# emdgroup/tnmf

Measured on AMD Instinct MI355X. Metric: MU-iterations/sec, higher is better.
Workload: dtype f32

## Files before the change

### tnmf_amd/csrc/fft.h

```cpp
#pragma once
#include "common.h"

struct FftArgs {
    const void *src0, *src1, *src2;
    void *dst0, *dst1;
    long ps_src, ps_dst;
    int planes, rows, cols;
    int ld_src, ld_dst;
    int KX, KXP;
    int yoff, xoff;
    int N, M, C, Hy;
    int n0, ngroups, nper;
    int mgroups, mper;
    int clamp0;
    double reg;
};

enum FftOp {
    kFftRowsFwd = 0,
    kFftRowsInv,
    kFftRowsInv2,
    kFftRowsMu,
    kFftColsFwd,
    kFftColsInv,
    kFftContractR,
    kFftGradH,
    kFftGradW,
};

typedef int (*fft_run_fn)(int op, int dtype, const FftArgs *a, hipStream_t s);
#define TNMF_FFT_DECL(L) int fft_run_##L(int op, int dtype, const FftArgs *a, hipStream_t s)
TNMF_FFT_DECL(32);
TNMF_FFT_DECL(48);
TNMF_FFT_DECL(64);
TNMF_FFT_DECL(96);
TNMF_FFT_DECL(144);
TNMF_FFT_DECL(192);
TNMF_FFT_DECL(270);
TNMF_FFT_DECL(288);
TNMF_FFT_DECL(384);
TNMF_FFT_DECL(540);
TNMF_FFT_DECL(576);
#undef TNMF_FFT_DECL

bool mixed_has_reconstruct(const Geo &g, int dtype);
bool mixed_has_grad_W(const Geo &g, int dtype);
int mixed_reconstruct(const Geo &g, const void *Tsp, const void *WT, void *OT, int KX, int KXP, hipStream_t s);
int mixed_grad_W(const Geo &g, const void *Tsp, const void *VT, const void *RT, void *Gn, void *Gp, int KX, int KXP,
                 int ngroups, int nper, hipStream_t s);

#ifndef TNMF_MIX_W3_WAVES
#define TNMF_MIX_W3_WAVES 3
#endif
constexpr int kMixW3Atoms = 16, kMixW3Waves = TNMF_MIX_W3_WAVES, kMixW3MaxAy = 12;
constexpr long kMixW3MinBytes = 24L << 20;
constexpr int mix_w3_waves(int Ay) {
    const int w = Ay >= 8 ? 3 : (Ay >= 4 ? 4 : (Ay >= 2 ? 5 : 7));
    return kMixW3Waves < 3 ? kMixW3Waves : w;
}
bool mixed_grad_W3_takes(const Geo &g, int KXP);

int spectral_contract_R(const Geo &g, int dtype, const void *SH, const void *SW, void *SR, int Ly, int KX, int KXP,
                        hipStream_t s);
int spectral_grad_W(const Geo &g, int dtype, const void *SH, const void *SV, const void *SR, void *Gn, void *Gp, int Ly,
                    int KX, int KXP, int ngroups, int nper, hipStream_t s);

bool fft_has(const Geo &g, int dtype);
void fft_invalidate(tnmf_hip_ctx *ctx);
void fft_invalidate_H(tnmf_hip_ctx *ctx, const Geo &g, int dtype, const void *H);
void fft_bind(tnmf_hip_ctx *ctx, const Geo &g, int dtype, const void *H, const void *V);
void fft_unbind(tnmf_hip_ctx *ctx);
void fft_invalidate_W(tnmf_hip_ctx *ctx);
void fft_release(tnmf_hip_ctx *ctx);
int fft_reserve(tnmf_hip_ctx *ctx, const Geo &g, int dtype, bool with_window);

int fft_reconstruct(tnmf_hip_ctx *ctx, const Geo &g, int dtype, const void *W, const void *H, void *R, bool nonneg,
                    hipStream_t s);
int fft_grad_H(tnmf_hip_ctx *ctx, const Geo &g, int dtype, const void *V, const void *R, const void *W, void *neg,
               void *pos, hipStream_t s);
int fft_update_H(tnmf_hip_ctx *ctx, const Geo &g, int dtype, const void *V, const void *R, const void *W, void *H,
                 double reg, hipStream_t s);
int fft_grad_W(tnmf_hip_ctx *ctx, const Geo &g, int dtype, const void *V, const void *R, const void *H, void *neg,
               void *pos, bool nonneg, hipStream_t s);
```

### tnmf_amd/csrc/fft.hip

```cpp
#include <algorithm>
#include <cstdlib>

#include "fft.h"
#include "fft_engine.h"

namespace {

const int kLensY[] = {32, 48, 64, 96, 144, 192, 270, 288, 384, 576};
const int kLensX[] = {32, 48, 64, 96, 144, 192, 270, 288, 384, 540, 576};
constexpr int kMixMaxGroups = 128;

int pick_len(int h, int dtype, bool along_x, bool tall = false) {
    if (along_x || tall) {
        for (int L : kLensX)
            if (L >= h && (dtype == 0 || L <= 288)) return L;
        return 0;
    }
    for (int L : kLensY)
        if (L >= h && (dtype == 0 || L <= 288)) return L;
    return 0;
}

bool tall_columns(const tnmf_hip_ctx *ctx) { return ctx->path != TNMF_PATH_FFT; }

fft_run_fn lookup(int L) {
    switch (L) {
        case 32: return fft_run_32;
        case 48: return fft_run_48;
        case 64: return fft_run_64;
        case 96: return fft_run_96;
        case 144: return fft_run_144;
        case 192: return fft_run_192;
        case 270: return fft_run_270;
        case 288: return fft_run_288;
        case 384: return fft_run_384;
        case 540: return fft_run_540;
        case 576: return fft_run_576;
        default: return nullptr;
    }
}

bool use_mixed(const Geo &g, int dtype, bool grad_W);

struct Lay {
    int Ly, Lx, KX, KXP, ngroups, nper, chunk, mgroups, mper;
    fft_run_fn rowf, colf;
    size_t csz;
    size_t T, SH, Tn, Tp, SV, SR, Ts, VT, RT, SW, SWf, TW, TWr, Wt, Gn, Gp, Gs, Wo, total, total_no_window;
    size_t sT, sSH, sS, sD;
    bool resident;
};

void sample_groups(const Geo &g, int tiles, int *ngroups, int *nper) {
    int ng = cdiv(2048, g.M * tiles);
    if (ng > 16) ng = 16;
    if (ng > g.N) ng = g.N;
    if (ng < 1) ng = 1;
    *nper = cdiv(g.N > 0 ? g.N : 1, ng);
    *ngroups = cdiv(g.N > 0 ? g.N : 1, *nper);
}

bool make_layout(const tnmf_hip_ctx *ctx, const Geo &gfull, const Geo &g, int dtype, Lay *l) {
    l->Ly = pick_len(g.Hy, dtype, false, tall_columns(ctx));
    l->Lx = pick_len(g.Hx, dtype, true);
    if (!l->Ly || !l->Lx) return false;
    l->rowf = lookup(l->Lx);
    l->colf = lookup(l->Ly);
    l->KX = l->Lx / 2 + 1;
    l->KXP = (int)align_up((size_t)l->KX, 16);
    l->csz = dtype == 0 ? 8 : 16;
    const int tiles = cdiv(l->KX, l->Ly > 384 ? 8 : 16);
    int ngroups_full, nper_full;
    sample_groups(gfull, tiles, &ngroups_full, &nper_full);
    sample_groups(g, tiles, &l->ngroups, &l->nper);
    const size_t c = l->csz, kxp = (size_t)l->KXP;
    const size_t Nf = gfull.N > 0 ? gfull.N : 1;
    l->sT = (size_t)g.M * g.Hy * kxp * c;
    l->sSH = (size_t)g.M * l->Ly * kxp * c;
    l->sS = (size_t)g.C * l->Ly * kxp * c;
    l->sD = (size_t)g.C * g.Dy * kxp * c;
    size_t budget = (size_t)8 << 30;
    if (const char *e = tnmf_diag_env("TNMF_FFT_WINDOW_MB")) budget = (size_t)atol(e) << 20;
    long chunk_full = (long)(budget / (2 * l->sT));
    if (chunk_full < 1) chunk_full = 1;
    if (chunk_full > (long)Nf) chunk_full = (long)Nf;
    l->chunk = (int)(chunk_full > g.N && g.N > 0 ? g.N : chunk_full);
    int mg = cdiv(1024, l->chunk * cdiv(l->KX, 16) * 2);
    if (mg > g.M) mg = g.M;
    if (mg < 1) mg = 1;
    l->mper = cdiv(g.M, mg);
    l->mgroups = cdiv(g.M, l->mper);
    const size_t nSW = (size_t)g.M * g.C * l->Ly * kxp * c;
    size_t o = 0;
    auto take = [&o](size_t bytes) {
        const size_t at = o;
        o += align_up(bytes, 256);
        return at;
    };
    l->T = take(Nf * l->sT + (size_t)64 * kxp * c);
    l->resident = !(use_mixed(g, dtype, false) && use_mixed(g, dtype, true));
    l->SH = take(l->resident ? Nf * l->sSH : 0);
    l->SV = take(Nf * l->sS);
    l->SR = take(Nf * l->sS);
    l->Ts = take(Nf * l->sD);
    l->VT = take(Nf * l->sD);
    l->RT = take(Nf * l->sD);
    l->SW = take(nSW);
    l->SWf = take(nSW);
    l->TW = take((size_t)2 * g.M * g.C * g.Ay * kxp * c);
    l->TWr = take((size_t)g.M * g.C * g.Ay * kxp * c);
    l->Wt = take((size_t)2 * g.M * g.C * g.Ay * g.Ax * (c / 2));
    const size_t nG = std::max(nSW * ngroups_full, (size_t)kMixMaxGroups * g.M * g.C * g.Ay * kxp * c);
    l->Gn = take(nG);
    l->Gp = take(nG);
    l->Gs = take(nSW * 2);
    l->Wo = take((size_t)2 * g.M * g.C * g.Ay * g.Ax * (c / 2));
    l->total_no_window = o;
    const size_t nTc = (size_t)chunk_full * l->sT;
    l->Tn = take(nTc);
    l->Tp = take(nTc);
    l->total = o;
    return true;
}

void clear_flags(FftState &f) {
    f.W_ok = false;
    std::fill(f.T_ok.begin(), f.T_ok.end(), 0);
    std::fill(f.SH_ok.begin(), f.SH_ok.end(), 0);
    std::fill(f.V_ok.begin(), f.V_ok.end(), 0);
    std::fill(f.SV_ok.begin(), f.SV_ok.end(), 0);
}

int ensure_ws(tnmf_hip_ctx *ctx, size_t bytes) {
    FftState &f = ctx->fft;
    if (bytes <= f.ws_bytes) return TNMF_OK;
    if (f.failed_bytes && bytes >= f.failed_bytes) return TNMF_E_WORKSPACE;
    const size_t want = align_up(bytes, 1 << 20);
    void *bigger = nullptr;
    if (hipMalloc(&bigger, want) != hipSuccess) {
        (void)hipGetLastError();
        bigger = nullptr;
        if (!f.ws) {
            f.failed_bytes = bytes;
            return TNMF_E_WORKSPACE;
        }
    }
    if (f.ws) {
        TNMF_HIP_TRY(hipDeviceSynchronize());
        TNMF_HIP_TRY(hipFree(f.ws));
        f.ws = nullptr;
        f.ws_bytes = 0;
        clear_flags(f);
    }
    if (!bigger && hipMalloc(&bigger, want) != hipSuccess) {
        (void)hipGetLastError();
        f.failed_bytes = bytes;
        return TNMF_E_WORKSPACE;
    }
    f.ws = bigger;
    f.ws_bytes = want;
    clear_flags(f);
    return TNMF_OK;
}

inline char *at(tnmf_hip_ctx *ctx, size_t off) { return static_cast<char *>(ctx->fft.ws) + off; }

#define CHECK(rc_expr)                  \
    do {                                \
        const int _rc = (rc_expr);      \
        if (_rc != TNMF_OK) return _rc; \
    } while (0)

template <typename T>
__global__ void k_fft_prep_W(const T *W, T *out0, T *out1, int planes, int Ay, int Ax, double scale) {
    const int i = blockIdx.x * blockDim.x + threadIdx.x, per = Ay * Ax;
    if (i >= planes * per) return;
    const int p = i / per, r = i - p * per, ay = r / Ax, ax = r - ay * Ax;
    const T v = (T)(scale * (double)W[i]);
    out0[i] = v;
    out1[(long)p * per + (Ay - 1 - ay) * Ax + (Ax - 1 - ax)] = v;
}

template <typename T>
__global__ __launch_bounds__(64) void k_fft_sum_groups(const cplx<T> *parts0, const cplx<T> *parts1, cplx<T> *out0,
                                                      cplx<T> *out1, long count, int ngroups, double scale) {
    const long i = (long)blockIdx.x * blockDim.x + threadIdx.x;
    if (i >= count) return;
    const cplx<T> *parts = blockIdx.y ? parts1 : parts0;
    double re = 0, im = 0;
    int gidx = 0;
    for (; gidx + 4 <= ngroups; gidx += 4) {
        cplx<T> v[4];
#pragma unroll
        for (int k = 0; k < 4; ++k) v[k] = parts[(gidx + k) * count + i];
#pragma unroll
        for (int k = 0; k < 4; ++k) {
            re += (double)v[k].x;
            im += (double)v[k].y;
        }
    }
    for (; gidx < ngroups; ++gidx) {
        const cplx<T> v = parts[gidx * count + i];
        re += (double)v.x;
        im += (double)v.y;
    }
    (blockIdx.y ? out1 : out0)[i] = {(T)(re * scale), (T)(im * scale)};
}

template <typename T>
__global__ void k_fft_flip_out(const T *in, T *out, int planes, int Ay, int Ax, int clamp0) {
    const int i = blockIdx.x * blockDim.x + threadIdx.x, per = Ay * Ax;
    if (i >= planes * per) return;
    const int p = i / per, r = i - p * per, ay = r / Ax, ax = r - ay * Ax;
    T v = in[(long)p * per + (Ay - 1 - ay) * Ax + (Ax - 1 - ax)];
    if (clamp0) v = v < (T)0 ? (T)0 : v;
    out[i] = v;
}

FftArgs base_args(const Geo &g, const Lay &l) {
    FftArgs a = {};
    a.KX = l.KX;
    a.KXP = l.KXP;
    a.N = g.N;
    a.M = g.M;
    a.C = g.C;
    a.Hy = g.Hy;
    return a;
}

int forward_planes(const Geo &g, const Lay &l, int dtype, const void *src, int planes, int rows, int cols, void *Ttmp,
                   void *S, hipStream_t s) {
    FftArgs a = base_args(g, l);
    a.src0 = src;
    a.dst0 = Ttmp;
    a.planes = planes;
    a.rows = rows;
    a.cols = cols;
    a.ld_src = cols;
    a.ps_src = (long)rows * cols;
    a.ps_dst = (long)rows * l.KXP;
    CHECK(l.rowf(kFftRowsFwd, dtype, &a, s));
    FftArgs b = base_args(g, l);
    b.src0 = Ttmp;
    b.dst0 = S;
    b.planes = planes;
    b.rows = rows;
    return l.colf(kFftColsFwd, dtype, &b, s);
}

bool use_mixed(const Geo &g, int dtype, bool grad_W) {
    static const bool off = tnmf_diag_env("TNMF_FFT_NO_MIXED") != nullptr;
    return !off && (grad_W ? mixed_has_grad_W(g, dtype) : mixed_has_reconstruct(g, dtype));
}

bool use_resident(const Lay &l) {
    static const bool off = tnmf_diag_env("TNMF_FFT_NO_RESIDENT") != nullptr;
    return l.resident && !off;
}

int scaled_W(tnmf_hip_ctx *ctx, const Geo &g, const Lay &l, int dtype, const void *W, double scale, hipStream_t s) {
    const int planes = g.M * g.C, n = planes * g.Ay * g.Ax;
    char *wt = at(ctx, l.Wt);
    const size_t half = (size_t)n * (l.csz / 2);
    if (dtype == 0)
        hipLaunchKernelGGL(k_fft_prep_W<float>, dim3(cdiv(n, 256)), dim3(256), 0, s, (const float *)W, (float *)wt,
                           (float *)(wt + half), planes, g.Ay, g.Ax, scale);
    else
        hipLaunchKernelGGL(k_fft_prep_W<double>, dim3(cdiv(n, 256)), dim3(256), 0, s, (const double *)W, (double *)wt,
                           (double *)(wt + half), planes, g.Ay, g.Ax, scale);
    TNMF_LAUNCH_CHECK();
    return TNMF_OK;
}

int spectra_W(tnmf_hip_ctx *ctx, const Geo &g, const Lay &l, int dtype, const void *W, bool plain, bool flipped,
              hipStream_t s) {
    const int planes = g.M * g.C, per = g.Ay * g.Ax, n = planes * per;
    const double scale = 1.0 / ((double)l.Ly * l.Lx);
    char *wt = at(ctx, l.Wt);
    const size_t half = (size_t)n * (l.csz / 2);
    if (dtype == 0)
        hipLaunchKernelGGL(k_fft_prep_W<float>, dim3(cdiv(n, 256)), dim3(256), 0, s, (const float *)W, (float *)wt,
                           (float *)(wt + half), planes, g.Ay, g.Ax, scale);
    else
        hipLaunchKernelGGL(k_fft_prep_W<double>, dim3(cdiv(n, 256)), dim3(256), 0, s, (const double *)W, (double *)wt,
                           (double *)(wt + half), planes, g.Ay, g.Ax, scale);
    TNMF_LAUNCH_CHECK();
    if (plain) CHECK(forward_planes(g, l, dtype, wt, planes, g.Ay, g.Ax, at(ctx, l.TW), at(ctx, l.SW), s));
    if (flipped) CHECK(forward_planes(g, l, dtype, wt + half, planes, g.Ay, g.Ax, at(ctx, l.TW), at(ctx, l.SWf), s));
    return TNMF_OK;
}


inline size_t esz_of(int dtype) { return dtype == 0 ? 4 : 8; }

bool same_shape(const Geo &a, const Geo &b) {
    return a.M == b.M && a.C == b.C && a.Dy == b.Dy && a.Dx == b.Dx && a.Ay == b.Ay && a.Ax == b.Ax && a.Hs == b.Hs;
}

void bind(FftState &f, const Geo &g, int dtype, const void *H, const void *V, bool explicit_bind) {
// ... 361 lines not shown
        CHECK(grad_H_window(ctx, g, c, dtype, n0, cnt, s));
        FftArgs a = base_args(g, l);
        a.src0 = at(ctx, l.Tn);
        a.src1 = at(ctx, l.Tp);
        a.dst0 = static_cast<char *>(H) + (size_t)n0 * hplane * esz;
        a.dst1 = c.T + (size_t)n0 * l.sT;
        a.planes = cnt * g.M;
        a.rows = g.Hy;
        a.cols = g.Hx;
        a.ld_dst = g.Hs;
        a.ps_src = (long)g.Hy * g.Hs;
        a.ps_dst = (long)g.Hy * l.KXP;
        a.reg = reg;
        CHECK(l.rowf(kFftRowsMu, dtype, &a, s));
    }
    if (track) set_ok(f.T_ok, c.sl.n0, g.N, 1);
    return TNMF_OK;
}

int mix_groups(const tnmf_hip_ctx *ctx, const Geo &g, const Lay &l) {
    const long slots = 2L * 4 * (ctx->num_cu > 0 ? ctx->num_cu : 256);
    const long per_group_block = (long)(g.C == 1 && g.Ay <= 12 ? cdiv(g.M, 2) : g.M) * cdiv(l.KX, 16);
    int best = 32;
    double best_cost = 1e30;
    for (int cand = 32; cand <= kMixMaxGroups; cand *= 2) {
        int ng = g.N < cand ? g.N : cand;
        const int nper = cdiv(g.N, ng);
        ng = cdiv(g.N, nper);
        const double rounds = (double)(per_group_block * cdiv(ng, 4)) / (double)slots;
        const double whole = rounds <= 1.0 ? 1.0 : (double)(long)(rounds + 0.999999);
        const double cost = whole / rounds + 0.03 * (cand / 32);
        if (cost < best_cost - 1e-9) {
            best_cost = cost;
            best = cand;
        }
    }
    return best;
}

int mix_groups_w3(const tnmf_hip_ctx *ctx, const Geo &g, const Lay &l) {
    const long slots3 = (long)mix_w3_waves(g.Ay) * (ctx->num_cu > 0 ? ctx->num_cu : 256);
    const long per_group = (long)cdiv(g.M, kMixW3Atoms) * cdiv(l.KX, 16);
    int best = 1;
    double best_cost = 1e30;
    for (int cand = g.N < kMixMaxGroups ? g.N : kMixMaxGroups; cand >= 1; --cand) {
        const int ng = cdiv(g.N, cdiv(g.N, cand));
        const double rounds = (double)(per_group * ng) / (double)slots3;
        const double whole = rounds <= 1.0 ? 1.0 : (double)(long)(rounds + 0.999999);
        const double cost3 = whole / rounds + 0.03 * ng / 32.0;
        if (cost3 < best_cost - 1e-9) {
            best_cost = cost3;
            best = ng;
        }
    }
    return best;
}

int fft_grad_W(tnmf_hip_ctx *ctx, const Geo &g, int dtype, const void *V, const void *R, const void *H, void *neg,
               void *pos, bool nonneg, hipStream_t s) {
    Call c;
    CHECK(prepare(ctx, g, dtype, H, V, &c));
    const Lay &l = c.l;
    CHECK(rows_of_H(ctx, g, c, dtype, H, s));
    const bool mixed = use_mixed(g, dtype, true);
    CHECK(spectra_V(ctx, g, c, dtype, V, !mixed, s));
    const int planes = 2 * g.M * g.C;
    if (mixed) {
        CHECK(forward_rows(g, l, dtype, R, g.N * g.C, g.Dy, g.Dx, c.RT, s));
        int ng_want = mix_groups(ctx, g, l);
        if (const char *e = tnmf_diag_env("TNMF_MIX_GROUPS")) ng_want = atoi(e);
        ng_want = ng_want < 1 ? 1 : (ng_want > kMixMaxGroups ? kMixMaxGroups : ng_want);
        int ng = g.N < ng_want ? g.N : ng_want;
        const int nper = cdiv(g.N, ng);
        ng = cdiv(g.N, nper);
        const int ngpad = (int)align_up((size_t)ng, 4);
        int nparts = ngpad, nper_call = nper;
        if (mixed_grad_W3_takes(g, l.KXP)) {
            nper_call = cdiv(g.N, mix_groups_w3(ctx, g, l));
            nparts = cdiv(g.N, nper_call);
        }
        CHECK(mixed_grad_W(g, c.T, c.VT, c.RT, at(ctx, l.Gn), at(ctx, l.Gp), l.KX, l.KXP, nparts, nper_call, s));
        const long count = (long)g.M * g.C * g.Ay * l.KXP;
        char *out = at(ctx, l.TW);
        hipLaunchKernelGGL(k_fft_sum_groups<float>, dim3((unsigned)((count + 63) / 64), 2), dim3(64), 0, s,
                           (const cplx<float> *)at(ctx, l.Gn), (const cplx<float> *)at(ctx, l.Gp), (cplx<float> *)out,
                           (cplx<float> *)(out + (size_t)count * l.csz), count, nparts, 1.0 / l.Lx);
        TNMF_LAUNCH_CHECK();
    } else {
        CHECK(forward_planes(g, l, dtype, R, g.N * g.C, g.Dy, g.Dx, c.Ts, c.SR, s));
        int ngroups = l.ngroups;
        if (use_resident(l)) {
            CHECK(spectra_of_H(ctx, g, c, dtype, H, s));
            const long blocks = (long)cdiv(g.M, 4) * (((long)l.Ly * l.KXP + 255) / 256) * cdiv(g.C, 4);
            int ng = (int)((8L * ctx->num_cu + blocks - 1) / blocks);
            ng = ng < 1 ? 1 : (ng > l.ngroups ? l.ngroups : ng);
            const int nper = cdiv(g.N, ng);
            ngroups = cdiv(g.N, nper);
            CHECK(spectral_grad_W(g, dtype, c.SH, c.SV, c.SR, at(ctx, l.Gn), at(ctx, l.Gp), l.Ly, l.KX, l.KXP, ngroups,
                                  nper, s));
        } else {
            FftArgs a = base_args(g, l);
            a.src0 = c.T;
            a.src1 = c.SV;
            a.src2 = c.SR;
            a.dst0 = at(ctx, l.Gn);
            a.dst1 = at(ctx, l.Gp);
            a.ngroups = l.ngroups;
            a.nper = l.nper;
            CHECK(l.colf(kFftGradW, dtype, &a, s));
        }
        const long count = (long)g.M * g.C * l.Ly * l.KXP;
        const size_t sbytes = (size_t)count * l.csz;
        const double scale = 1.0 / ((double)l.Ly * l.Lx);
        {
            char *out = at(ctx, l.Gs);
            const dim3 grid((unsigned)((count + 63) / 64), 2);
            if (dtype == 0)
                hipLaunchKernelGGL(k_fft_sum_groups<float>, grid, dim3(64), 0, s, (const cplx<float> *)at(ctx, l.Gn),
                                   (const cplx<float> *)at(ctx, l.Gp), (cplx<float> *)out, (cplx<float> *)(out + sbytes),
                                   count, ngroups, scale);
            else
                hipLaunchKernelGGL(k_fft_sum_groups<double>, grid, dim3(64), 0, s, (const cplx<double> *)at(ctx, l.Gn),
                                   (const cplx<double> *)at(ctx, l.Gp), (cplx<double> *)out,
                                   (cplx<double> *)(out + sbytes), count, ngroups, scale);
            TNMF_LAUNCH_CHECK();
        }
        FftArgs b = base_args(g, l);
        b.src0 = at(ctx, l.Gs);
        b.dst0 = at(ctx, l.TW);
        b.planes = planes;
        b.rows = g.Ay;
        b.yoff = 0;
        CHECK(l.colf(kFftColsInv, dtype, &b, s));
    }
    FftArgs d = base_args(g, l);
    d.src0 = at(ctx, l.TW);
    d.dst0 = at(ctx, l.Wo);
    d.planes = planes;
    d.rows = g.Ay;
    d.cols = g.Ax;
    d.xoff = 0;
    d.ld_dst = g.Ax;
    d.ps_dst = (long)g.Ay * g.Ax;
    CHECK(l.rowf(kFftRowsInv, dtype, &d, s));
    const int per = g.M * g.C * g.Ay * g.Ax;
    const char *wo = at(ctx, l.Wo);
    if (dtype == 0) {
        hipLaunchKernelGGL(k_fft_flip_out<float>, dim3(cdiv(per, 256)), dim3(256), 0, s, (const float *)wo,
                           (float *)neg, g.M * g.C, g.Ay, g.Ax, nonneg ? 1 : 0);
        hipLaunchKernelGGL(k_fft_flip_out<float>, dim3(cdiv(per, 256)), dim3(256), 0, s, (const float *)wo + per,
                           (float *)pos, g.M * g.C, g.Ay, g.Ax, nonneg ? 1 : 0);
    } else {
        hipLaunchKernelGGL(k_fft_flip_out<double>, dim3(cdiv(per, 256)), dim3(256), 0, s, (const double *)wo,
                           (double *)neg, g.M * g.C, g.Ay, g.Ax, nonneg ? 1 : 0);
        hipLaunchKernelGGL(k_fft_flip_out<double>, dim3(cdiv(per, 256)), dim3(256), 0, s, (const double *)wo + per,
                           (double *)pos, g.M * g.C, g.Ay, g.Ax, nonneg ? 1 : 0);
    }
    TNMF_LAUNCH_CHECK();
    return TNMF_OK;
}
```

### tnmf_amd/csrc/fft_kernels.h

```cpp
#pragma once
#include <atomic>
#include "fft.h"
#include "fft_engine.h"
#include "fft_len_twiddles.h"

namespace {


template <int L>
struct LenCfg {
    static constexpr int col_tile = L > 384 ? 8 : 16;
    static constexpr int col_threads = (L == 270 || L == 540) ? 480 : (L > 192 ? 512 : 256);
    static_assert((L * col_tile) % col_threads == 0 && (L * 16) % col_threads == 0, "whole tile elements per thread");
    static constexpr int col_elems = L * col_tile / col_threads;
    static constexpr int row_pairs = L > 288 ? 8 : 16;
    static constexpr int row_threads = 256;
    static constexpr int mu_pairs = L > 288 ? 4 : 8;
    static constexpr int mu_threads = L / 2 + 1 > 256 ? 512 : 256;
};

template <int L, bool WIDE>
struct ColTile {
    static constexpr int v = WIDE ? 16 : LenCfg<L>::col_tile;
};

template <typename T, int L>
__device__ __forceinline__ void make_twiddles(cplx<T> *tw, int tid, int nt) {
    static_assert(sizeof(tnmf_len_twiddles) == sizeof(double) * 2 * L, "the table of this translation unit's length");
    for (int t = tid; t < L; t += nt) tw[t] = {(T)tnmf_len_twiddles[t][0], (T)tnmf_len_twiddles[t][1]};
}

template <typename T, typename P, int NB, int BS, int NT>
__device__ __forceinline__ void tile_fwd(cplx<T> *x, const cplx<T> *tw, int tid) {
#pragma unroll 1
    for (int t = tid; t < NB * P::tasks1; t += NT) P::template fwd1<BS>(x + (t % NB), tw, t / NB);
    __syncthreads();
#pragma unroll 1
    for (int t = tid; t < NB * P::tasks2; t += NT) P::template fwd2<BS>(x + (t % NB), tw, t / NB);
    __syncthreads();
#pragma unroll 1
    for (int t = tid; t < NB * P::tasks3; t += NT) P::template fwd3<BS>(x + (t % NB), t / NB);
    __syncthreads();
}

template <typename T, typename P, int NB, int BS, int NT>
__device__ __forceinline__ void tile_inv(cplx<T> *x, const cplx<T> *tw, int tid) {
#pragma unroll 1
    for (int t = tid; t < NB * P::tasks3; t += NT) P::template inv3<BS>(x + (t % NB), t / NB);
    __syncthreads();
#pragma unroll 1
    for (int t = tid; t < NB * P::tasks2; t += NT) P::template inv2<BS>(x + (t % NB), tw, t / NB);
    __syncthreads();
#pragma unroll 1
    for (int t = tid; t < NB * P::tasks1; t += NT) P::template inv1<BS>(x + (t % NB), tw, t / NB);
    __syncthreads();
}


template <typename T, typename P, int NB, int BS, int NT>
__device__ __forceinline__ void store_rows_split(const cplx<T> *x, cplx<T> *dst, int y0, int rows, int KXP, int tid) {
    constexpr int L = P::L, KX = L / 2 + 1;
    for (int idx = tid; idx < 2 * NB * KX; idx += NT) {
        const int r = idx / KX, k = idx - r * KX, y = y0 + r;
        if (y >= rows) continue;
        const int pr = r >> 1;
        const cplx<T> z1 = x[P::pos_of_k(k) * BS + pr];
        const cplx<T> z2 = x[P::pos_of_k(k == 0 ? 0 : L - k) * BS + pr];
        cplx<T> A, B;
        split_pair(z1, z2, A, B);
        dst[(long)y * KXP + k] = (r & 1) ? B : A;
    }
}

template <typename T, typename P, int NB, int BS, int NT>
__device__ __forceinline__ void load_rows_merge(cplx<T> *x, const cplx<T> *src, int y0, int rows, int KXP, int tid) {
    constexpr int L = P::L, KX = L / 2 + 1;
    for (int idx = tid; idx < NB * KX; idx += NT) {
        const int pr = idx / KX, k = idx - pr * KX, ya = y0 + 2 * pr;
        cplx<T> A = {0, 0}, B = {0, 0};
        if (ya < rows) A = src[(long)ya * KXP + k];
        if (ya + 1 < rows) B = src[(long)(ya + 1) * KXP + k];
        if (k == 0 || 2 * k == L) {
            x[P::pos_of_k(k) * BS + pr] = {A.x, B.x};
        } else {
            cplx<T> zk, zlk;
            merge_pair(A, B, zk, zlk);
            x[P::pos_of_k(k) * BS + pr] = zk;
            x[P::pos_of_k(L - k) * BS + pr] = zlk;
        }
    }
}

template <typename T, int L, int NB, int NT>
__global__ __launch_bounds__(NT) void k_fft_rows_fwd(FftArgs a) {
    using P = FftPlanFor<T, L>;
    constexpr int BS = NB + 1, KX = L / 2 + 1, R2 = 2 * NB;
    constexpr int XS = (L + NT - 1) / NT, KS = (KX + NT - 1) / NT;
    extern __shared__ __align__(16) unsigned char smem[];
    cplx<T> *x = reinterpret_cast<cplx<T> *>(smem);
    cplx<T> *tw = x + L * BS;
    const int tid = threadIdx.x, y0 = blockIdx.x * R2;
    const long plane = blockIdx.y;
    make_twiddles<T, L>(tw, tid, NT);
    const T *src = static_cast<const T *>(a.src0) + plane * a.ps_src;
    T *xr = reinterpret_cast<T *>(x);
    if (tid < L) {
        const int xc = min(tid, a.cols - 1);
        T v[R2];
#pragma unroll
        for (int r = 0; r < R2; ++r) v[r] = src[(long)min(y0 + r, a.rows - 1) * a.ld_src + xc];
#pragma unroll
        for (int r = 0; r < R2; ++r) xr[tid * (2 * BS) + r] = (y0 + r < a.rows && tid < a.cols) ? v[r] : (T)0;
    }
    if constexpr (XS > 2) {
#pragma unroll
        for (int sl = 1; sl < XS; ++sl) {
            const int xx = tid + sl * NT;
            if (xx < L) {
                const int xc = min(xx, a.cols - 1);
                T v[R2];
#pragma unroll
                for (int r = 0; r < R2; ++r) v[r] = src[(long)min(y0 + r, a.rows - 1) * a.ld_src + xc];
#pragma unroll
                for (int r = 0; r < R2; ++r) xr[xx * (2 * BS) + r] = (y0 + r < a.rows && xx < a.cols) ? v[r] : (T)0;
            }
        }
    } else if constexpr (XS == 2) {
        const int rem = a.cols > NT ? a.cols - NT : 0, c0 = NT + rem;
        for (int idx = tid; idx < rem * R2; idx += NT) {
            const int r = idx / rem, c = idx - r * rem;
            xr[(NT + c) * (2 * BS) + r] = y0 + r < a.rows ? src[(long)(y0 + r) * a.ld_src + NT + c] : (T)0;
        }
        for (int idx = tid; idx < (L - c0) * R2; idx += NT) {
            const int c = idx / R2, r = idx - c * R2;
            xr[(c0 + c) * (2 * BS) + r] = (T)0;
        }
    }
    __syncthreads();
    tile_fwd<T, P, NB, BS, NT>(x, tw, tid);
    cplx<T> *dst = static_cast<cplx<T> *>(a.dst0) + plane * a.ps_dst;
#pragma unroll
    for (int ks = 0; ks < KS; ++ks) {
        const int k = tid + ks * NT;
        if (k < KX) {
            const int pk = P::pos_of_k(k) * BS, plk = P::pos_of_k(k == 0 ? 0 : L - k) * BS;
#pragma unroll
            for (int p = 0; p < NB; ++p) {
                const int ya = y0 + 2 * p;
                cplx<T> A, B;
                split_pair(x[pk + p], x[plk + p], A, B);
                if (ya < a.rows) dst[(long)ya * a.KXP + k] = A;
                if (ya + 1 < a.rows) dst[(long)(ya + 1) * a.KXP + k] = B;
            }
        }
    }
}

template <typename T, int L, int NB, int NT, int MODE>
__global__ __launch_bounds__(NT) void k_fft_rows_inv(FftArgs a) {
    using P = FftPlanFor<T, L>;
    constexpr int BS = NB + 1;
    extern __shared__ __align__(16) unsigned char smem[];
    cplx<T> *x = reinterpret_cast<cplx<T> *>(smem);
    cplx<T> *xb = x + L * BS;
    cplx<T> *tw = MODE == 0 ? xb : xb + L * BS;
    const int tid = threadIdx.x, y0 = blockIdx.x * 2 * NB;
    const long plane = blockIdx.y;
    make_twiddles<T, L>(tw, tid, NT);
    const long tin = plane * ((long)a.rows * a.KXP);
    load_rows_merge<T, P, NB, BS, NT>(x, static_cast<const cplx<T> *>(a.src0) + tin, y0, a.rows, a.KXP, tid);
    if (MODE != 0)
        load_rows_merge<T, P, NB, BS, NT>(xb, static_cast<const cplx<T> *>(a.src1) + tin, y0, a.rows, a.KXP, tid);
    __syncthreads();
    tile_inv<T, P, NB, BS, NT>(x, tw, tid);
    if (MODE != 0) tile_inv<T, P, NB, BS, NT>(xb, tw, tid);
    const T *xr = reinterpret_cast<const T *>(x);
    const T *xbr = reinterpret_cast<const T *>(xb);
    T *d0 = static_cast<T *>(a.dst0) + plane * a.ps_dst;
    T *d1 = MODE == 1 ? static_cast<T *>(a.dst1) + plane * a.ps_dst : nullptr;
    for (int idx = tid; idx < 2 * NB * a.cols; idx += NT) {
        const int r = idx / a.cols, xc = idx - r * a.cols, y = y0 + r;
        if (y >= a.rows) continue;
        const int off = ((xc + a.xoff) * BS + (r >> 1)) * 2 + (r & 1);
        T v = xr[off];
        if (MODE == 0 && a.clamp0) v = v < (T)0 ? (T)0 : v;
        d0[(long)y * a.ld_dst + xc] = v;
        if (MODE == 1) d1[(long)y * a.ld_dst + xc] = xbr[off];
    }
}

template <typename T, int L, int NB, int NT>
__global__ __launch_bounds__(NT) void k_fft_rows_mu(FftArgs a) {
    using P = FftPlanFor<T, L>;
    constexpr int BS = NB + 1, KX = L / 2 + 1, R2 = 2 * NB;
    constexpr int XS = (L + NT - 1) / NT;
    constexpr int KS = (KX + NT - 1) / NT;
    static_assert(KS == 1, "block size must cover Lx/2+1 frequencies");
    extern __shared__ __align__(16) unsigned char smem[];
    cplx<T> *x = reinterpret_cast<cplx<T> *>(smem);
    cplx<T> *tw = x + L * BS;
    T *stash = reinterpret_cast<T *>(tw + L);
    T *xr = reinterpret_cast<T *>(x);
    const int tid = threadIdx.x, y0 = blockIdx.x * R2;
    const long plane = blockIdx.y;
    make_twiddles<T, L>(tw, tid, NT);
    const long tin = plane * ((long)a.rows * a.KXP);
    const cplx<T> *sn = static_cast<const cplx<T> *>(a.src0) + tin;
    const cplx<T> *sp = static_cast<const cplx<T> *>(a.src1) + tin;
    T *Hp = static_cast<T *>(a.dst0) + plane * a.ps_src;
    const int k = tid < KX ? tid : KX - 1;
    const bool kact = tid < KX;
    const int pk = P::pos_of_k(k) * BS, plk = P::pos_of_k(k == 0 ? 0 : L - k) * BS;
    const bool kself = (k == 0 || 2 * k == L);
    cplx<T> na[NB], nb[NB], pa[NB], pb[NB];
#pragma unroll
    for (int p = 0; p < NB; ++p) {
        na[p] = sn[(long)min(y0 + 2 * p, a.rows - 1) * a.KXP + k];
        nb[p] = sn[(long)min(y0 + 2 * p + 1, a.rows - 1) * a.KXP + k];
    }
#pragma unroll
    for (int p = 0; p < NB; ++p) {
        pa[p] = sp[(long)min(y0 + 2 * p, a.rows - 1) * a.KXP + k];
        pb[p] = sp[(long)min(y0 + 2 * p + 1, a.rows - 1) * a.KXP + k];
    }
    const int xc = min(tid, a.cols - 1);
    T hv[R2];
#pragma unroll
    for (int r = 0; r < R2; ++r) hv[r] = Hp[(long)min(y0 + r, a.rows - 1) * a.ld_dst + xc];
    if (kact) {
#pragma unroll
        for (int p = 0; p < NB; ++p) {
            const int ya = y0 + 2 * p;
            cplx<T> A = na[p], B = nb[p];
            if (ya >= a.rows) A = {0, 0};
            if (ya + 1 >= a.rows) B = {0, 0};
            if (kself) {
                x[pk + p] = {A.x, B.x};
            } else {
                cplx<T> zk, zlk;
                merge_pair(A, B, zk, zlk);
                x[pk + p] = zk;
                x[plk + p] = zlk;
            }
        }
    }
    __syncthreads();
    tile_inv<T, P, NB, BS, NT>(x, tw, tid);
    T ng[R2];
    if (tid < L) {
#pragma unroll
        for (int r = 0; r < R2; ++r) ng[r] = xr[tid * (2 * BS) + r];
    }
#pragma unroll
    for (int sl = 1; sl < XS; ++sl) {
        const int xx = tid + sl * NT;
        if (xx < L) {
#pragma unroll
            for (int r = 0; r < R2; ++r) stash[(xx - NT) * R2 + r] = xr[xx * (2 * BS) + r];
        }
    }
    __syncthreads();
    if (kact) {
#pragma unroll
        for (int p = 0; p < NB; ++p) {
            const int ya = y0 + 2 * p;
            cplx<T> A = pa[p], B = pb[p];
            if (ya >= a.rows) A = {0, 0};
            if (ya + 1 >= a.rows) B = {0, 0};
            if (kself) {
                x[pk + p] = {A.x, B.x};
// ... 319 lines not shown
        for (int e = 0; e < E; ++e) {
            const int idx = tid + e * NT, pos = idx / ColTile<L, WIDE>::v, col = idx % ColTile<L, WIDE>::v;
            const cplx<T> h = x[pos * (ColTile<L, WIDE>::v + 1) + col];
            if (PRE) {
                cfmac(an[0][e], h, v[PRE ? e : 0]);
                cfmac(ap[0][e], h, r[PRE ? e : 0]);
            } else {
#pragma unroll
                for (int cc = 0; cc < CG; ++cc) {
                    const long pl = ((long)n * a.C + min(c0 + cc, a.C - 1)) * splane;
                    const unsigned o = (unsigned)(pos * a.KXP + ln.kxc);
                    cfmac(an[cc][e], h, (SV + pl)[o]);
                    cfmac(ap[cc][e], h, (SR + pl)[o]);
                }
            }
        }
        __syncthreads();
    }
    cplx<T> *Gn = static_cast<cplx<T> *>(a.dst0) + (long)grp * a.M * a.C * splane;
    cplx<T> *Gp = static_cast<cplx<T> *>(a.dst1) + (long)grp * a.M * a.C * splane;
#pragma unroll
    for (int cc = 0; cc < CG; ++cc) {
        if (c0 + cc >= a.C) continue;
#pragma unroll
        for (int e = 0; e < E; ++e) {
            const int idx = tid + e * NT, pos = idx / ColTile<L, WIDE>::v, col = idx % ColTile<L, WIDE>::v, kx = kx0 + col;
            if (kx < a.KX) {
                const long o = ((long)m * a.C + c0 + cc) * splane + (long)pos * a.KXP + kx;
                Gn[o] = an[cc][e];
                Gp[o] = ap[cc][e];
            }
        }
    }
}


template <typename K>
int set_lds_limit(K kernel, size_t bytes) {
    if (bytes > 64 * 1024) TNMF_HIP_TRY(hipFuncSetAttribute((const void *)kernel,
                                                           hipFuncAttributeMaxDynamicSharedMemorySize, 160 * 1024));
    return TNMF_OK;
}

#define TNMF_FFT_LAUNCH(kernel, grid, threads, lds)                         \
    do {                                                                    \
        static std::atomic<unsigned long long> attr_done{0};                \
        int dev_ = 0;                                                       \
        TNMF_HIP_TRY(hipGetDevice(&dev_));                                  \
        const unsigned long long bit_ = 1ull << (dev_ & 63);                \
        if (!(attr_done.load(std::memory_order_acquire) & bit_)) {          \
             \
                                             \
            const int _rc = set_lds_limit(kernel, (lds));                   \
            if (_rc != TNMF_OK) return _rc;                                 \
            attr_done.fetch_or(bit_, std::memory_order_release);            \
        }                                                                   \
        hipLaunchKernelGGL(kernel, grid, dim3(threads), (lds), s, *a);      \
        TNMF_LAUNCH_CHECK();                                                \
        return TNMF_OK;                                                     \
    } while (0)

template <typename T, int L>
int fft_run_typed(int op, const FftArgs *a, hipStream_t s) {
    using Cfg = LenCfg<L>;
    constexpr int NB = (sizeof(T) == 8 && L > 144) ? Cfg::row_pairs / 2 : Cfg::row_pairs;
    constexpr int NTR = Cfg::row_threads, NTC = Cfg::col_threads;
    constexpr size_t row_tile = (size_t)L * (NB + 1) * sizeof(cplx<T>), tw_bytes = (size_t)L * sizeof(cplx<T>);
    constexpr size_t col_lds = (size_t)L * (LenCfg<L>::col_tile + 1) * sizeof(cplx<T>) + tw_bytes;
    constexpr size_t wide_lds = (size_t)L * 17 * sizeof(cplx<T>) + tw_bytes;
    if (row_tile * 2 + tw_bytes > 160 * 1024 || col_lds > 160 * 1024 || wide_lds > 160 * 1024) return TNMF_E_UNSUPPORTED;
    FftArgs flat;
    if ((op == kFftRowsFwd || op == kFftRowsInv) && a->rows == 1 && a->planes > 1) {
        flat = *a;
        flat.rows = a->planes;
        flat.planes = 1;
        a = &flat;
    }
    const dim3 rgrid((unsigned)cdiv(a->rows, 2 * NB), (unsigned)a->planes);
    const unsigned tiles = (unsigned)cdiv(a->KX, LenCfg<L>::col_tile), wide_tiles = (unsigned)cdiv(a->KX, 16);
    switch (op) {
        case kFftRowsFwd: TNMF_FFT_LAUNCH((k_fft_rows_fwd<T, L, NB, NTR>), rgrid, NTR, row_tile + tw_bytes);
        case kFftRowsInv: TNMF_FFT_LAUNCH((k_fft_rows_inv<T, L, NB, NTR, 0>), rgrid, NTR, row_tile + tw_bytes);
        case kFftRowsInv2: TNMF_FFT_LAUNCH((k_fft_rows_inv<T, L, NB, NTR, 1>), rgrid, NTR, 2 * row_tile + tw_bytes);
        case kFftRowsMu: {
            constexpr int NBM = (sizeof(T) == 8 && L > 144) ? Cfg::mu_pairs / 2 : Cfg::mu_pairs;
            const dim3 mgrid((unsigned)cdiv(a->rows, 2 * NBM), (unsigned)a->planes);
            constexpr int NTM = Cfg::mu_threads;
            constexpr size_t stash = L > NTM ? (size_t)(L - NTM) * 2 * NBM * sizeof(T) : 0;
            TNMF_FFT_LAUNCH((k_fft_rows_mu<T, L, NBM, NTM>), mgrid, NTM,
                            (size_t)L * (NBM + 1) * sizeof(cplx<T>) + tw_bytes + stash);
        }
        case kFftColsFwd:
            TNMF_FFT_LAUNCH((k_fft_cols_fwd<T, L, NTC>), dim3(tiles, (unsigned)a->planes), NTC, col_lds);
        case kFftColsInv:
            TNMF_FFT_LAUNCH((k_fft_cols_inv<T, L, NTC>), dim3(tiles, (unsigned)a->planes), NTC, col_lds);
        case kFftContractR: {
            const int cg = a->C <= 3 ? a->C : 4;
            const dim3 grid((unsigned)a->N, tiles, (unsigned)cdiv(a->C, cg));
            if (cg == 1) TNMF_FFT_LAUNCH((k_fft_contract_R<T, L, NTC, 1>), grid, NTC, col_lds);
            if (cg == 2) TNMF_FFT_LAUNCH((k_fft_contract_R<T, L, NTC, 2>), grid, NTC, col_lds);
            if (cg == 3) TNMF_FFT_LAUNCH((k_fft_contract_R<T, L, NTC, 3>), grid, NTC, col_lds);
            TNMF_FFT_LAUNCH((k_fft_contract_R<T, L, NTC, 4>), grid, NTC, col_lds);
        }
        case kFftGradH: {
            const dim3 grid((unsigned)a->planes, wide_tiles, 2u * (unsigned)a->mgroups);
            if (a->C == 1) TNMF_FFT_LAUNCH((k_fft_grad_H<T, L, NTC, 1>), grid, NTC, wide_lds);
            if (a->C == 2) TNMF_FFT_LAUNCH((k_fft_grad_H<T, L, NTC, 2>), grid, NTC, wide_lds);
            if (a->C == 3) TNMF_FFT_LAUNCH((k_fft_grad_H<T, L, NTC, 3>), grid, NTC, wide_lds);
            if (a->C == 4) TNMF_FFT_LAUNCH((k_fft_grad_H<T, L, NTC, 4>), grid, NTC, wide_lds);
            TNMF_FFT_LAUNCH((k_fft_grad_H<T, L, NTC, 0>), grid, NTC, wide_lds);
        }
        case kFftGradW: {
            const int cg = a->C <= 2 ? a->C : (Cfg::col_elems <= 9 ? 3 : 2);
            const dim3 grid((unsigned)a->M, tiles, (unsigned)(a->ngroups * cdiv(a->C, cg)));
            if (cg == 1) TNMF_FFT_LAUNCH((k_fft_grad_W<T, L, NTC, 1>), grid, NTC, col_lds);
            if (cg == 2) TNMF_FFT_LAUNCH((k_fft_grad_W<T, L, NTC, 2>), grid, NTC, col_lds);
            TNMF_FFT_LAUNCH((k_fft_grad_W<T, L, NTC, 3>), grid, NTC, col_lds);
        }
        default: break;
    }
    return TNMF_E_UNSUPPORTED;
}

}
```

Baseline: 216.9.

## Fuse W-gradient flip into inverse row FFT and restructure row load/store bursts

Adds a flip mode to the inverse row FFT kernel that writes neg/pos planes directly with reversed row/column indexing and optional clamp. This removes the Wo scratch buffer and two separate flip kernels. The inverse row kernel also gets burst-batched loads in load_rows_merge and column-per-thread burst stores. The group-sum kernel now uses 256 threads and a 16-wide unroll. The new paths add register pressure and strided reversed stores.

```diff
diff --git a/tnmf_amd/csrc/fft.h b/tnmf_amd/csrc/fft.h
--- a/tnmf_amd/csrc/fft.h
+++ b/tnmf_amd/csrc/fft.h
@@ -26,6 +26,7 @@
     kFftContractR,
     kFftGradH,
     kFftGradW,
+    kFftRowsInvFlip,
 };
 
 typedef int (*fft_run_fn)(int op, int dtype, const FftArgs *a, hipStream_t s);
diff --git a/tnmf_amd/csrc/fft.hip b/tnmf_amd/csrc/fft.hip
--- a/tnmf_amd/csrc/fft.hip
+++ b/tnmf_amd/csrc/fft.hip
@@ -46,7 +46,7 @@
     int Ly, Lx, KX, KXP, ngroups, nper, chunk, mgroups, mper;
     fft_run_fn rowf, colf;
     size_t csz;
-    size_t T, SH, Tn, Tp, SV, SR, Ts, VT, RT, SW, SWf, TW, TWr, Wt, Gn, Gp, Gs, Wo, total, total_no_window;
+    size_t T, SH, Tn, Tp, SV, SR, Ts, VT, RT, SW, SWf, TW, TWr, Wt, Gn, Gp, Gs, total, total_no_window;
     size_t sT, sSH, sS, sD;
     bool resident;
 };
@@ -114,7 +114,6 @@
     l->Gn = take(nG);
     l->Gp = take(nG);
     l->Gs = take(nSW * 2);
-    l->Wo = take((size_t)2 * g.M * g.C * g.Ay * g.Ax * (c / 2));
     l->total_no_window = o;
     const size_t nTc = (size_t)chunk_full * l->sT;
     l->Tn = take(nTc);
@@ -181,40 +180,36 @@
     out1[(long)p * per + (Ay - 1 - ay) * Ax + (Ax - 1 - ax)] = v;
 }
 
+constexpr int kSumGroupsThreads = 256;
+
+template <typename T, int U>
+__device__ __forceinline__ void sum_groups_burst(const cplx<T> *parts, long count, long i, int &gidx, int ngroups,
+                                                 double &re, double &im) {
+    for (; gidx + U <= ngroups; gidx += U) {
+        cplx<T> v[U];
+#pragma unroll
+        for (int k = 0; k < U; ++k) v[k] = parts[(gidx + k) * count + i];
+#pragma unroll
+        for (int k = 0; k < U; ++k) {
+            re += (double)v[k].x;
+            im += (double)v[k].y;
+        }
+    }
+}
+
 template <typename T>
-__global__ __launch_bounds__(64) void k_fft_sum_groups(const cplx<T> *parts0, const cplx<T> *parts1, cplx<T> *out0,
-                                                      cplx<T> *out1, long count, int ngroups, double scale) {
+__global__ __launch_bounds__(kSumGroupsThreads) void k_fft_sum_groups(const cplx<T> *parts0, const cplx<T> *parts1,
+                                                                     cplx<T> *out0, cplx<T> *out1, long count,
+                                                                     int ngroups, double scale) {
     const long i = (long)blockIdx.x * blockDim.x + threadIdx.x;
     if (i >= count) return;
     const cplx<T> *parts = blockIdx.y ? parts1 : parts0;
     double re = 0, im = 0;
     int gidx = 0;
-    for (; gidx + 4 <= ngroups; gidx += 4) {
-        cplx<T> v[4];
-#pragma unroll
-        for (int k = 0; k < 4; ++k) v[k] = parts[(gidx + k) * count + i];
-#pragma unroll
-        for (int k = 0; k < 4; ++k) {
-            re += (double)v[k].x;
-            im += (double)v[k].y;
-        }
-    }
-    for (; gidx < ngroups; ++gidx) {
-        const cplx<T> v = parts[gidx * count + i];
-        re += (double)v.x;
-        im += (double)v.y;
-    }
+    sum_groups_burst<T, 16>(parts, count, i, gidx, ngroups, re, im);
+    sum_groups_burst<T, 4>(parts, count, i, gidx, ngroups, re, im);
+    sum_groups_burst<T, 1>(parts, count, i, gidx, ngroups, re, im);
     (blockIdx.y ? out1 : out0)[i] = {(T)(re * scale), (T)(im * scale)};
-}
-
-template <typename T>
-__global__ void k_fft_flip_out(const T *in, T *out, int planes, int Ay, int Ax, int clamp0) {
-    const int i = blockIdx.x * blockDim.x + threadIdx.x, per = Ay * Ax;
-    if (i >= planes * per) return;
-    const int p = i / per, r = i - p * per, ay = r / Ax, ax = r - ay * Ax;
-    T v = in[(long)p * per + (Ay - 1 - ay) * Ax + (Ax - 1 - ax)];
-    if (clamp0) v = v < (T)0 ? (T)0 : v;
-    out[i] = v;
 }
 
 FftArgs base_args(const Geo &g, const Lay &l) {
@@ -742,7 +737,8 @@
         CHECK(mixed_grad_W(g, c.T, c.VT, c.RT, at(ctx, l.Gn), at(ctx, l.Gp), l.KX, l.KXP, nparts, nper_call, s));
         const long count = (long)g.M * g.C * g.Ay * l.KXP;
         char *out = at(ctx, l.TW);
-        hipLaunchKernelGGL(k_fft_sum_groups<float>, dim3((unsigned)((count + 63) / 64), 2), dim3(64), 0, s,
+        hipLaunchKernelGGL(k_fft_sum_groups<float>, dim3((unsigned)((count + kSumGroupsThreads - 1) / kSumGroupsThreads), 2),
+                           dim3(kSumGroupsThreads), 0, s,
                            (const cplx<float> *)at(ctx, l.Gn), (const cplx<float> *)at(ctx, l.Gp), (cplx<float> *)out,
                            (cplx<float> *)(out + (size_t)count * l.csz), count, nparts, 1.0 / l.Lx);
         TNMF_LAUNCH_CHECK();
@@ -774,13 +770,15 @@
         const double scale = 1.0 / ((double)l.Ly * l.Lx);
         {
             char *out = at(ctx, l.Gs);
-            const dim3 grid((unsigned)((count + 63) / 64), 2);
+            const dim3 grid((unsigned)((count + kSumGroupsThreads - 1) / kSumGroupsThreads), 2);
             if (dtype == 0)
-                hipLaunchKernelGGL(k_fft_sum_groups<float>, grid, dim3(64), 0, s, (const cplx<float> *)at(ctx, l.Gn),
+                hipLaunchKernelGGL(k_fft_sum_groups<float>, grid, dim3(kSumGroupsThreads), 0, s,
+                                   (const cplx<float> *)at(ctx, l.Gn),
                                    (const cplx<float> *)at(ctx, l.Gp), (cplx<float> *)out, (cplx<float> *)(out + sbytes),
                                    count, ngroups, scale);
             else
-                hipLaunchKernelGGL(k_fft_sum_groups<double>, grid, dim3(64), 0, s, (const cplx<double> *)at(ctx, l.Gn),
+                hipLaunchKernelGGL(k_fft_sum_groups<double>, grid, dim3(kSumGroupsThreads), 0, s,
+                                   (const cplx<double> *)at(ctx, l.Gn),
                                    (const cplx<double> *)at(ctx, l.Gp), (cplx<double> *)out,
                                    (cplx<double> *)(out + sbytes), count, ngroups, scale);
             TNMF_LAUNCH_CHECK();
@@ -795,27 +793,14 @@
     }
     FftArgs d = base_args(g, l);
     d.src0 = at(ctx, l.TW);
-    d.dst0 = at(ctx, l.Wo);
+    d.dst0 = neg;
+    d.dst1 = pos;
     d.planes = planes;
     d.rows = g.Ay;
     d.cols = g.Ax;
     d.xoff = 0;
     d.ld_dst = g.Ax;
     d.ps_dst = (long)g.Ay * g.Ax;
-    CHECK(l.rowf(kFftRowsInv, dtype, &d, s));
-    const int per = g.M * g.C * g.Ay * g.Ax;
-    const char *wo = at(ctx, l.Wo);
-    if (dtype == 0) {
-        hipLaunchKernelGGL(k_fft_flip_out<float>, dim3(cdiv(per, 256)), dim3(256), 0, s, (const float *)wo,
-                           (float *)neg, g.M * g.C, g.Ay, g.Ax, nonneg ? 1 : 0);
-        hipLaunchKernelGGL(k_fft_flip_out<float>, dim3(cdiv(per, 256)), dim3(256), 0, s, (const float *)wo + per,
-                           (float *)pos, g.M * g.C, g.Ay, g.Ax, nonneg ? 1 : 0);
-    } else {
-        hipLaunchKernelGGL(k_fft_flip_out<double>, dim3(cdiv(per, 256)), dim3(256), 0, s, (const double *)wo,
-                           (double *)neg, g.M * g.C, g.Ay, g.Ax, nonneg ? 1 : 0);
-        hipLaunchKernelGGL(k_fft_flip_out<double>, dim3(cdiv(per, 256)), dim3(256), 0, s, (const double *)wo + per,
-                           (double *)pos, g.M * g.C, g.Ay, g.Ax, nonneg ? 1 : 0);
-    }
-    TNMF_LAUNCH_CHECK();
-    return TNMF_OK;
-}
+    d.clamp0 = nonneg ? 1 : 0;
+    return l.rowf(kFftRowsInvFlip, dtype, &d, s);
+}
diff --git a/tnmf_amd/csrc/fft_kernels.h b/tnmf_amd/csrc/fft_kernels.h
--- a/tnmf_amd/csrc/fft_kernels.h
+++ b/tnmf_amd/csrc/fft_kernels.h
@@ -72,23 +72,54 @@
     }
 }
 
-template <typename T, typename P, int NB, int BS, int NT>
+template <typename T, typename P, int NB, int BS, int NT, int PB>
 __device__ __forceinline__ void load_rows_merge(cplx<T> *x, const cplx<T> *src, int y0, int rows, int KXP, int tid) {
-    constexpr int L = P::L, KX = L / 2 + 1;
-    for (int idx = tid; idx < NB * KX; idx += NT) {
-        const int pr = idx / KX, k = idx - pr * KX, ya = y0 + 2 * pr;
-        cplx<T> A = {0, 0}, B = {0, 0};
-        if (ya < rows) A = src[(long)ya * KXP + k];
-        if (ya + 1 < rows) B = src[(long)(ya + 1) * KXP + k];
-        if (k == 0 || 2 * k == L) {
-            x[P::pos_of_k(k) * BS + pr] = {A.x, B.x};
-        } else {
-            cplx<T> zk, zlk;
-            merge_pair(A, B, zk, zlk);
-            x[P::pos_of_k(k) * BS + pr] = zk;
-            x[P::pos_of_k(L - k) * BS + pr] = zlk;
-        }
-    }
+    constexpr int L = P::L, KX = L / 2 + 1, KS = (KX + NT - 1) / NT;
+    static_assert(NB % PB == 0, "whole bursts");
+#pragma unroll
+    for (int ks = 0; ks < KS; ++ks) {
+        if ((tid & ~63) + ks * NT >= KX) continue;
+        const int kk = tid + ks * NT, k = kk < KX ? kk : KX - 1;
+        const int pk = P::pos_of_k(k) * BS, plk = P::pos_of_k(k == 0 ? 0 : L - k) * BS;
+        const bool kself = (k == 0 || 2 * k == L);
+#pragma unroll
+        for (int p0 = 0; p0 < NB; p0 += PB) {
+            cplx<T> va[PB], vb[PB];
+#pragma unroll
+            for (int p = 0; p < PB; ++p) {
+                va[p] = src[(long)min(y0 + 2 * (p0 + p), rows - 1) * KXP + k];
+                vb[p] = src[(long)min(y0 + 2 * (p0 + p) + 1, rows - 1) * KXP + k];
+            }
+            if (kk < KX) {
+#pragma unroll
+                for (int p = 0; p < PB; ++p) {
+                    const int ya = y0 + 2 * (p0 + p);
+                    cplx<T> A = va[p], B = vb[p];
+                    if (ya >= rows) A = {0, 0};
+                    if (ya + 1 >= rows) B = {0, 0};
+                    if (kself) {
+                        x[pk + p0 + p] = {A.x, B.x};
+                    } else {
+                        cplx<T> zk, zlk;
+                        merge_pair(A, B, zk, zlk);
+                        x[pk + p0 + p] = zk;
+                        x[plk + p0 + p] = zlk;
+                    }
+                }
+            }
+            __builtin_amdgcn_sched_barrier(0);
+        }
+    }
+}
+
+template <typename T, int L, int NB, int MODE>
+constexpr int rows_inv_burst() {
+    constexpr long lds = (long)(MODE == 1 ? 2 : 1) * L * (NB + 1) * sizeof(cplx<T>) + (long)L * sizeof(cplx<T>);
+    constexpr int by_lds = (int)(160 * 1024 / lds), waves = by_lds > 8 ? 8 : (by_lds < 1 ? 1 : by_lds);
+    constexpr int budget = 512 / waves / 8 * 8 - 24;
+    int pb = NB;
+    while (pb > 1 && pb * (int)sizeof(T) > budget) pb /= 2;
+    return pb;
 }
 
 template <typename T, int L, int NB, int NT>
@@ -159,33 +190,62 @@
 template <typename T, int L, int NB, int NT, int MODE>
 __global__ __launch_bounds__(NT) void k_fft_rows_inv(FftArgs a) {
     using P = FftPlanFor<T, L>;
-    constexpr int BS = NB + 1;
+    constexpr int BS = NB + 1, R2 = 2 * NB, CS = (L + NT - 1) / NT;
     extern __shared__ __align__(16) unsigned char smem[];
     cplx<T> *x = reinterpret_cast<cplx<T> *>(smem);
     cplx<T> *xb = x + L * BS;
-    cplx<T> *tw = MODE == 0 ? xb : xb + L * BS;
+    cplx<T> *tw = MODE != 1 ? xb : xb + L * BS;
     const int tid = threadIdx.x, y0 = blockIdx.x * 2 * NB;
     const long plane = blockIdx.y;
     make_twiddles<T, L>(tw, tid, NT);
     const long tin = plane * ((long)a.rows * a.KXP);
-    load_rows_merge<T, P, NB, BS, NT>(x, static_cast<const cplx<T> *>(a.src0) + tin, y0, a.rows, a.KXP, tid);
-    if (MODE != 0)
-        load_rows_merge<T, P, NB, BS, NT>(xb, static_cast<const cplx<T> *>(a.src1) + tin, y0, a.rows, a.KXP, tid);
+    constexpr int PB = rows_inv_burst<T, L, NB, MODE>();
+    load_rows_merge<T, P, NB, BS, NT, PB>(x, static_cast<const cplx<T> *>(a.src0) + tin, y0, a.rows, a.KXP, tid);
+    if (MODE == 1)
+        load_rows_merge<T, P, NB, BS, NT, PB>(xb, static_cast<const cplx<T> *>(a.src1) + tin, y0, a.rows, a.KXP, tid);
     __syncthreads();
     tile_inv<T, P, NB, BS, NT>(x, tw, tid);
-    if (MODE != 0) tile_inv<T, P, NB, BS, NT>(xb, tw, tid);
+    if (MODE == 1) tile_inv<T, P, NB, BS, NT>(xb, tw, tid);
     const T *xr = reinterpret_cast<const T *>(x);
     const T *xbr = reinterpret_cast<const T *>(xb);
-    T *d0 = static_cast<T *>(a.dst0) + plane * a.ps_dst;
-    T *d1 = MODE == 1 ? static_cast<T *>(a.dst1) + plane * a.ps_dst : nullptr;
-    for (int idx = tid; idx < 2 * NB * a.cols; idx += NT) {
-        const int r = idx / a.cols, xc = idx - r * a.cols, y = y0 + r;
-        if (y >= a.rows) continue;
-        const int off = ((xc + a.xoff) * BS + (r >> 1)) * 2 + (r & 1);
-        T v = xr[off];
-        if (MODE == 0 && a.clamp0) v = v < (T)0 ? (T)0 : v;
-        d0[(long)y * a.ld_dst + xc] = v;
-        if (MODE == 1) d1[(long)y * a.ld_dst + xc] = xbr[off];
+    const long half = a.planes / 2;
+    const bool second = MODE == 2 && plane >= half;
+    T *d0 = static_cast<T *>(second ? a.dst1 : a.dst0) + (second ? plane - half : plane) * a.ps_dst;
+    T *d1 = MODE == 1 ? static_cast<T *>(a.dst1) + plane * a.ps_dst : d0;
+    const long rs = MODE == 2 ? -(long)a.ld_dst : (long)a.ld_dst;
+    const int cs = MODE == 2 ? -1 : 1;
+    const long q00 = MODE == 2 ? (long)(a.rows - 1 - y0) * a.ld_dst + (a.cols - 1) : (long)y0 * a.ld_dst;
+#pragma unroll
+    for (int st = 0; st <= (MODE == 1 ? 1 : 0); ++st) {
+        const T *xs = st == 0 ? xr : xbr;
+        T *q = (st == 0 ? d0 : d1) + q00;
+        const bool clamp = MODE != 1 && a.clamp0;
+#pragma unroll
+        for (int sl = 0; sl < CS; ++sl) {
+            const int xc = tid + sl * NT;
+            if (xc < a.cols) {
+                const int off = (xc + a.xoff) * (2 * BS);
+#pragma unroll
+                for (int r0 = 0; r0 < R2; r0 += 2 * PB) {
+                    T v[2 * PB];
+#pragma unroll
+                    for (int r = 0; r < 2 * PB; ++r) v[r] = xs[off + r0 + r];
+                    if (clamp) {
+#pragma unroll
+                        for (int r = 0; r < 2 * PB; ++r) v[r] = v[r] < (T)0 ? (T)0 : v[r];
+                    }
+                    if (y0 + r0 + 2 * PB <= a.rows) {
+#pragma unroll
+                        for (int r = 0; r < 2 * PB; ++r) q[(r0 + r) * rs + xc * cs] = v[r];
+                    } else {
+#pragma unroll
+                        for (int r = 0; r < 2 * PB; ++r)
+                            if (y0 + r0 + r < a.rows) q[(r0 + r) * rs + xc * cs] = v[r];
+                    }
+                    __builtin_amdgcn_sched_barrier(0);
+                }
+            }
+        }
     }
 }
 
@@ -671,6 +731,7 @@
         case kFftRowsFwd: TNMF_FFT_LAUNCH((k_fft_rows_fwd<T, L, NB, NTR>), rgrid, NTR, row_tile + tw_bytes);
         case kFftRowsInv: TNMF_FFT_LAUNCH((k_fft_rows_inv<T, L, NB, NTR, 0>), rgrid, NTR, row_tile + tw_bytes);
         case kFftRowsInv2: TNMF_FFT_LAUNCH((k_fft_rows_inv<T, L, NB, NTR, 1>), rgrid, NTR, 2 * row_tile + tw_bytes);
+        case kFftRowsInvFlip: TNMF_FFT_LAUNCH((k_fft_rows_inv<T, L, NB, NTR, 2>), rgrid, NTR, row_tile + tw_bytes);
         case kFftRowsMu: {
             constexpr int NBM = (sizeof(T) == 8 && L > 144) ? Cfg::mu_pairs / 2 : Cfg::mu_pairs;
             const dim3 mgrid((unsigned)cdiv(a->rows, 2 * NBM), (unsigned)a->planes);
```

New measurement: 218.3 (median of 6 runs). No clear change (+0.7%).
